# MarSaKi/VLN-BEVBert

Measured on AMD Instinct MI355X. Metric: pretrain_samples_per_sec, higher is better.
Workload: dtype bf16+fp32-residual

## Files before the change

include/bevbert_hip.h:

```cpp
#ifndef BEVBERT_HIP_H
#define BEVBERT_HIP_H

#include <stdint.h>

#ifdef __cplusplus
extern "C" {
#endif

typedef struct ihipStream_t* hipStream_t;

#define BEVBERT_F32 0
#define BEVBERT_BF16 1
#define BEVBERT_F16 2

const char* bevbert_last_error(void);
int bevbert_version(void);
int bevbert_hip_error_reset(void);
const char* bevbert_arch(void);
const char* bevbert_attn_last_path(int backward);
const char* bevbert_attn_plan(int B, int nh, int Lq, int Lk, int dtype, int impl, int has_key_mask, int has_bias,
                              float drop_p, int has_bits, int bits_ready, int want_dbias, int ncu, int backward);

int bevbert_bev_lift_bin(const float* depths, const float* T_c2w, const float* T_w2c, const float* S_w2c,
                         const float* pix_scale, int B, int V, int hw, float depth_scale, int dim, float res,
// ... 29 lines not shown
int bevbert_layernorm_bwd(const void* dy, const void* z, const float* mean, const float* rstd, const float* gamma,
                          void* dz, void* dx, float* dgamma, float* dbeta, float* dbias, float* workspace, int rows,
                          int H, int dtype, float drop_p, uint64_t seed, uint64_t offset, int accumulate,
                          hipStream_t stream);
int bevbert_layernorm_bwd_add(const void* dy, const void* z, const float* mean, const float* rstd, const float* gamma,
                              void* dz, void* dx, const void* dz_add, float* dgamma, float* dbeta, float* dbias,
                              float* workspace, int rows, int H, int dtype, float drop_p, uint64_t seed, uint64_t offset,
                              int accumulate, hipStream_t stream);
int bevbert_layernorm_res32_fwd(const void* x, const float* bias, const void* residual, int residual_dtype,
                                const float* gamma, const float* beta, void* y16, float* y32, float* z32, float* mean,
                                float* rstd, int rows, int H, float eps, float drop_p, uint64_t seed, uint64_t offset,
                                hipStream_t stream);
int bevbert_layernorm_res32_bwd(const void* dy16, const float* dy32, const float* z32, const float* mean,
                                const float* rstd, const float* gamma, void* dz, void* dx16, float* dgamma,
                                float* dbeta, float* dbias, float* workspace, int rows, int H, float drop_p, uint64_t seed,
                                uint64_t offset, int accumulate, int dz_dtype,
                                hipStream_t stream);
int64_t bevbert_colsum_workspace_floats(int total_cols);
int bevbert_colsum_partial_rows(int rows);
int bevbert_colsum_finalize(const float* partials, int nblocks, int nwhich, int C, float* out0, float* out1,
                            float* out2, int accumulate, hipStream_t stream);
int bevbert_colsum_partials(const void* dy, float* partials, int rows, int C, int dtype, hipStream_t stream);
int bevbert_multi_finalize(const void* tasks, int ntasks, hipStream_t stream);
int bevbert_multi_accum(const void* tasks, int ntasks, hipStream_t stream);

int bevbert_embed_sum_layernorm_fwd(const int64_t* ids, const void* word, const void* pos, const void* type_row,
                                    const float* gamma, const float* beta, void* y, void* z_out, float* mean,
                                    float* rstd, int rows, int L, int H, float eps, int dtype, float drop_p,
                                    uint64_t seed, uint64_t offset, hipStream_t stream);

int bevbert_embedding_grad(const int64_t* ids, const void* d, float* table_grad, int rows, int H, int padding_idx,
                           int dtype, hipStream_t stream);

int64_t bevbert_smallk_workspace_floats(int rows, int K, int H);
int bevbert_smallk_linear_layernorm_fwd(const float* feat, const float* weight, const float* bias, const float* gamma,
                                        const float* beta, const void* post1, const void* table, const int64_t* idx,
                                        void* y, float* mean, float* rstd, int rows, int K, int H, float eps, int dtype,
                                        hipStream_t stream);
int bevbert_smallk_linear_layernorm_bwd(const void* dy, const float* feat, const float* weight, const float* bias,
                                        const float* mean, const float* rstd, const float* gamma, float* dweight,
                                        float* dbias, float* dgamma, float* dbeta, float* workspace, int rows, int K,
                                        int H, int dtype, hipStream_t stream);

int bevbert_colsum_any(const void* dy, float* out, int rows, int C, int dtype, int accumulate, hipStream_t stream);

int bevbert_weighted_mean_fwd(const float* x, const float* w, const float* denom_dev, float denom, int n, float* out,
                              hipStream_t stream);
int bevbert_weighted_mean_bwd(const float* dout, const float* w, const float* denom_dev, float denom, int n, float* dx,
                              hipStream_t stream);

int bevbert_sem_select(const uint8_t* mask1, const uint8_t* mask2, int n, int cap, int classes, int64_t* idx, float* valid,
                       float* denom, hipStream_t stream);
int bevbert_bce_rows_fwd(const void* logits, const uint8_t* labels, const int64_t* idx, float* out, int rows, int C, int dtype,
                         hipStream_t stream);
int bevbert_bce_rows_bwd(const void* logits, const uint8_t* labels, const int64_t* idx, const float* g, void* dlogits, int rows,
                         int C, int dtype, hipStream_t stream);

int bevbert_graph_bias_fwd(const float* dists, const float* w, const float* b, float* out, int64_t n, hipStream_t stream);
int bevbert_graph_bias_bwd(const float* dbias, const float* dists, int layers, int B, int nh, int G, float* dw, float* db,
                           float* workspace , hipStream_t stream);

int bevbert_rows_gather(const void* src, const int64_t* ids, void* out, int rows, int H, int dtype, hipStream_t stream);
int bevbert_rows_scatter(const int64_t* ids, const void* d, void* out, int rows, int H, int dtype, int accumulate,
                         hipStream_t stream);

int bevbert_embedding_grad_sliced(const int64_t* ids, const void* d, float* partials, int rows, int H, int table_rows,
// ... 139 lines not shown
```

vln_bevbert_amd/csrc/rowops.hip:

```cpp
#include <math.h>
#include <type_traits>

#include "common.h"

template <typename T, int NV, bool GATHER>
__global__ __launch_bounds__(256) void ln_fwd_kernel(const T* __restrict__ x, const float* __restrict__ bias,
                                                     const T* __restrict__ residual, const float* __restrict__ gamma,
                                                     const float* __restrict__ beta, T* __restrict__ y,
                                                     T* __restrict__ z_out, float* __restrict__ mean_out,
                                                     float* __restrict__ rstd_out, int rows, float eps, float drop_p,
                                                     uint32_t drop_thr, uint32_t drop_key,
                                                     const int64_t* __restrict__ ids, const T* __restrict__ word,
                                                     const T* __restrict__ pos, const T* __restrict__ type_row, int L,
                                                     const uint32_t* __restrict__ salt) {
  constexpr int H = NV * 256;
  if (drop_p > 0.f) drop_key = bb_salted(drop_key, salt);
  const int lane = threadIdx.x & 63;
  const int row = blockIdx.x * 4 + (threadIdx.x >> 6);
  if (row >= rows) return;
  float4 v[NV];
  const float keep_scale = drop_p > 0.f ? 1.0f / (1.0f - drop_p) : 1.0f;
#pragma unroll
  for (int i = 0; i < NV; ++i) {
    const int col = (i * 64 + lane) * 4;
// ... 466 lines not shown
  const int r = blockIdx.x;
  const int e0 = rowptr[r], e1 = rowptr[r + 1];
  for (int c = threadIdx.x * 4; c < H; c += blockDim.x * 4) {
    float4 acc = make_float4(0.f, 0.f, 0.f, 0.f);
    for (int e = e0; e < e1; ++e) {
      const float ww = w[e];
      const float4 v = ld4<T>(src + (size_t)idx[e] * H + c);
      acc.x += ww * v.x; acc.y += ww * v.y; acc.z += ww * v.z; acc.w += ww * v.w;
    }
    st4<T>(out + (size_t)r * H + c, acc);
  }
}

template <typename T>
__global__ __launch_bounds__(256) void accum_partials_kernel(const T* __restrict__ partials, float* __restrict__ sink,
                                                             int S, size_t n4) {
  for (size_t i = (size_t)blockIdx.x * 256 + threadIdx.x; i < n4; i += (size_t)gridDim.x * 256) {
    float4 acc = *reinterpret_cast<const float4*>(sink + i * 4);
    for (int s = 0; s < S; ++s) {
      const float4 v = ld4<T>(partials + ((size_t)s * n4 + i) * 4);
      acc.x += v.x; acc.y += v.y; acc.z += v.z; acc.w += v.w;
    }
    *reinterpret_cast<float4*>(sink + i * 4) = acc;
  }
}

struct AccumTask {
  const void* partials;
  float* sink;
  unsigned long long n4_total;
  unsigned int off4, n4;
  int S, dtype;
};
template <typename T>
__device__ __forceinline__ void accum_task(const AccumTask& t) {
  const T* part = (const T*)t.partials;
  for (unsigned i = threadIdx.x; i < t.n4; i += 256) {
    float4 acc = *reinterpret_cast<const float4*>(t.sink + (size_t)i * 4);
    for (int s = 0; s < t.S; ++s) {
      const float4 v = ld4<T>(part + ((size_t)s * t.n4_total + t.off4 + i) * 4);
      acc.x += v.x; acc.y += v.y; acc.z += v.z; acc.w += v.w;
    }
    *reinterpret_cast<float4*>(t.sink + (size_t)i * 4) = acc;
  }
}
__global__ __launch_bounds__(256) void multi_accum_kernel(const AccumTask* __restrict__ tasks) {
  const AccumTask t = tasks[blockIdx.x];
  if (t.dtype == BB_BF16) accum_task<bf16_raw>(t);
  else accum_task<float>(t);
}

#define EG_MAXJ 4
template <typename T, typename TO = float, bool ACCUM = true>
__global__ __launch_bounds__(256) void embedding_grad_kernel(const int64_t* __restrict__ ids, const T* __restrict__ d,
                                                             TO* __restrict__ table_grad, int rows, int H,
                                                             int padding_idx) {
  __shared__ int s_flag;
  __shared__ float s_part[4][256 * EG_MAXJ];
  const int r = blockIdx.x, tid = threadIdx.x, lane = tid & 63, wave = tid >> 6;
  const int64_t id = ids[r];
  if (id == (int64_t)padding_idx) return;
  if (tid == 0) s_flag = 0;
  __syncthreads();
  int hit = 0;
  for (int i = tid; i < r; i += 256) hit |= (ids[i] == id);
  if (hit) s_flag = 1;
  __syncthreads();
  if (s_flag) return;
  float4 acc[EG_MAXJ];
#pragma unroll
  for (int j = 0; j < EG_MAXJ; ++j) acc[j] = make_float4(0.f, 0.f, 0.f, 0.f);
  const int span = rows - r, q = (span + 3) >> 2;
  const int lo = r + wave * q, hi = min(rows, lo + q);
  for (int base = lo; base < hi; base += 256) {
    unsigned long long bal[4];
#pragma unroll
    for (int u = 0; u < 4; ++u) {
      const int i = base + 64 * u + lane;
      bal[u] = __ballot(i < hi && ids[i] == id);
    }
#pragma unroll
    for (int u = 0; u < 4; ++u) {
      unsigned long long b = bal[u];
      while (b) {
        const int row = base + 64 * u + (__ffsll((long long)b) - 1);
        b &= b - 1;
#pragma unroll
        for (int j = 0; j < EG_MAXJ; ++j) {
          const int c = (lane + 64 * j) * 4;
          if (c < H) {
            const float4 v = ld4<T>(d + (size_t)row * H + c);
            acc[j].x += v.x; acc[j].y += v.y; acc[j].z += v.z; acc[j].w += v.w;
          }
        }
      }
    }
  }
#pragma unroll
  for (int j = 0; j < EG_MAXJ; ++j) *reinterpret_cast<float4*>(&s_part[wave][(lane + 64 * j) * 4]) = acc[j];
  __syncthreads();
  TO* dst = table_grad + (size_t)id * H;
  for (int c = tid * 4; c < H; c += 1024) {
    const float4 p0 = *reinterpret_cast<const float4*>(&s_part[0][c]), p1 = *reinterpret_cast<const float4*>(&s_part[1][c]);
    const float4 p2 = *reinterpret_cast<const float4*>(&s_part[2][c]), p3 = *reinterpret_cast<const float4*>(&s_part[3][c]);
    float4 t = make_float4(0.f, 0.f, 0.f, 0.f);
    if (ACCUM) t = ld4<TO>(dst + c);
    t.x += (p0.x + p1.x) + (p2.x + p3.x); t.y += (p0.y + p1.y) + (p2.y + p3.y);
    t.z += (p0.z + p1.z) + (p2.z + p3.z); t.w += (p0.w + p1.w) + (p2.w + p3.w);
    st4<TO>(dst + c, t);
  }
}

template <typename T>
__global__ __launch_bounds__(256) void rows_gather_kernel(const T* __restrict__ src, const int64_t* __restrict__ ids,
                                                          T* __restrict__ out, int H) {
  const int64_t id = ids[blockIdx.x];
  for (int c = threadIdx.x * 4; c < H; c += blockDim.x * 4)
    st4<T>(out + (size_t)blockIdx.x * H + c, ld4<T>(src + (size_t)id * H + c));
}

template <typename T>
__global__ __launch_bounds__(256) void embedding_grad_sliced_kernel(const int64_t* __restrict__ ids, const T* __restrict__ d,
                                                                    float* __restrict__ partials, int rows, int H,
                                                                    int rows_per_slice, int ntab) {
  const int t = blockIdx.x, s = blockIdx.y;
  const int r0 = s * rows_per_slice, r1 = min(rows, r0 + rows_per_slice);
  for (int c = threadIdx.x * 4; c < H; c += blockDim.x * 4) {
    float4 acc = make_float4(0.f, 0.f, 0.f, 0.f);
    for (int r = r0; r < r1; r += 4) {
      float4 v[4];
#pragma unroll
      for (int j = 0; j < 4; ++j) {
        v[j] = make_float4(0.f, 0.f, 0.f, 0.f);
        if (r + j < r1 && ids[r + j] == t) v[j] = ld4<T>(d + (size_t)(r + j) * H + c);
      }
#pragma unroll
      for (int j = 0; j < 4; ++j) { acc.x += v[j].x; acc.y += v[j].y; acc.z += v[j].z; acc.w += v[j].w; }
    }
    *reinterpret_cast<float4*>(partials + ((size_t)s * ntab + t) * H + c) = acc;
  }
}

__global__ __launch_bounds__(256) void sumsq_kernel(const float* __restrict__ g, size_t n4, float* __restrict__ partials) {
// ... 731 lines not shown
    hipLaunchKernelGGL((embedding_grad_kernel<float, float, true>), dim3(rows), dim3(256), 0, stream, ids, (const float*)d, (float*)out, rows, H, -1);
  else if (dtype == BB_F32)
    hipLaunchKernelGGL((embedding_grad_kernel<float, float, false>), dim3(rows), dim3(256), 0, stream, ids, (const float*)d, (float*)out, rows, H, -1);
  else if (dtype == BB_BF16 && accumulate)
    hipLaunchKernelGGL((embedding_grad_kernel<bf16_raw, bf16_raw, true>), dim3(rows), dim3(256), 0, stream, ids, (const bf16_raw*)d, (bf16_raw*)out, rows, H, -1);
  else if (dtype == BB_BF16)
    hipLaunchKernelGGL((embedding_grad_kernel<bf16_raw, bf16_raw, false>), dim3(rows), dim3(256), 0, stream, ids, (const bf16_raw*)d, (bf16_raw*)out, rows, H, -1);
  else {
    bb_set_error("rows_scatter: dtype %d unsupported", dtype);
    return BB_EUNSUPPORTED;
  }
  BB_CHECK_LAUNCH("rows_scatter");
  return BB_OK;
}

BEVBERT_API int bevbert_embedding_grad(const int64_t* ids, const void* d, float* table_grad, int rows, int H,
                                       int padding_idx, int dtype, hipStream_t stream) {
  BB_REQUIRE(H % 4 == 0 && H <= 256 * EG_MAXJ, "embedding_grad: H=%d must be a multiple of 4 and <= %d", H, 256 * EG_MAXJ);
  if (rows <= 0) return BB_OK;
  if (dtype == BB_F32)
    hipLaunchKernelGGL(embedding_grad_kernel<float>, dim3(rows), dim3(256), 0, stream, ids, (const float*)d, table_grad, rows, H,
                       padding_idx);
  else if (dtype == BB_BF16)
    hipLaunchKernelGGL(embedding_grad_kernel<bf16_raw>, dim3(rows), dim3(256), 0, stream, ids, (const bf16_raw*)d, table_grad,
                       rows, H, padding_idx);
  else {
    bb_set_error("embedding_grad: dtype %d unsupported", dtype);
    return BB_EUNSUPPORTED;
  }
  BB_CHECK_LAUNCH("embedding_grad");
  return BB_OK;
}

BEVBERT_API int bevbert_embedding_grad_sliced(const int64_t* ids, const void* d, float* partials, int rows, int H,
                                              int table_rows, int rows_per_slice, int dtype, hipStream_t stream) {
  BB_REQUIRE(H % 4 == 0, "embedding_grad_sliced: H=%d must be a multiple of 4", H);
  BB_REQUIRE(table_rows > 0 && rows_per_slice > 0 && rows > 0, "embedding_grad_sliced: empty problem (%d table rows, %d rows)",
             table_rows, rows);
  const int slices = (rows + rows_per_slice - 1) / rows_per_slice;
  BB_REQUIRE(slices <= 65535, "embedding_grad_sliced: %d slices exceed the grid limit", slices);
  const int nt = H / 4 < 256 ? ((H / 4 + 63) / 64) * 64 : 256;
  const dim3 grid(table_rows, slices);
  if (dtype == BB_F32)
    hipLaunchKernelGGL(embedding_grad_sliced_kernel<float>, grid, dim3(nt), 0, stream, ids, (const float*)d, partials, rows, H,
                       rows_per_slice, table_rows);
  else if (dtype == BB_BF16)
    hipLaunchKernelGGL(embedding_grad_sliced_kernel<bf16_raw>, grid, dim3(nt), 0, stream, ids, (const bf16_raw*)d, partials,
                       rows, H, rows_per_slice, table_rows);
  else {
    bb_set_error("embedding_grad_sliced: dtype %d unsupported", dtype);
    return BB_EUNSUPPORTED;
  }
  BB_CHECK_LAUNCH("embedding_grad_sliced");
  return BB_OK;
}

BEVBERT_API int bevbert_grad_norm_clip(const float* grads, int64_t n, float pre_scale, float max_norm,
                                       float* partials, float* scalars, hipStream_t stream) {
  BB_REQUIRE(n % 4 == 0, "grad_norm_clip: n must be a multiple of 4");
  hipLaunchKernelGGL(sumsq_kernel, dim3(1024), dim3(256), 0, stream, grads, (size_t)n / 4, partials);
  hipLaunchKernelGGL(clip_coef_kernel, dim3(1), dim3(256), 0, stream, partials, 1024, pre_scale, max_norm, scalars);
  BB_CHECK_LAUNCH("grad_norm_clip");
  return BB_OK;
}

BEVBERT_API int bevbert_adamw_step(float* params, const float* grads, float* exp_avg, float* exp_avg_sq,
// ... 56 lines not shown
```

vln_bevbert_amd/lib.py:

```python
import ctypes
import os
import re
import subprocess

import torch

_HERE = os.path.dirname(os.path.abspath(__file__))
LIB_PATH = os.path.join(_HERE, "libbevbert_hip.so")
CSRC = os.path.join(_HERE, "csrc")
EXTRA_FLAGS = {"attn_fwd4.hip": ["-fno-slp-vectorize"]}
SOURCES = ["splat.hip", "rowops.hip", "attn_simple.hip", "attn_f32.hip", "attn_mfma.hip", "attn_bwd1.hip", "attn_fwd2.hip", "attn_fwd4.hip", "attn_bwd2.hip", "attn_bwd3.hip", "attn_small.hip", "attn_short.hip", "smallk.hip", "sap_loss.hip", "graph_nav.hip", "nav_expert.hip", "waypoint.hip", "gemm.hip", "capi.hip"]
HEADER = os.path.join(os.path.dirname(_HERE), "include", "bevbert_hip.h")

F32, BF16, F16 = 0, 1, 2
_DT = {torch.float32: F32, torch.bfloat16: BF16, torch.float16: F16}


class BevBertHipError(RuntimeError):
    pass


def dtype_code(t):
    try:
        return _DT[t.dtype if torch.is_tensor(t) else t]
# ... 30 lines not shown


def header_symbols():
    with open(HEADER) as f:
        return sorted(set(re.findall(r"\b(bevbert_\w+)\s*\(", f.read())))


_lib = None
_P, _I, _I64, _U64, _F = ctypes.c_void_p, ctypes.c_int, ctypes.c_int64, ctypes.c_uint64, ctypes.c_float

_PROTOS = {
    "bevbert_bev_lift_bin": [_P, _P, _P, _P, _P, _I, _I, _I, _F, _I, _F, _F, _P, _P, _P, _P],
    "bevbert_bev_bin_points": [_P, _P, _I, _I, _I, _F, _F, _P, _P, _P, _P],
    "bevbert_bev_splat_mean": [_P, _I, _P, _P, _P, _I, _I, _I, _I, _I, _P, _P, _I, _P, _P, _P, _I, _P],
    "bevbert_attn_fwd": [_P, _P, _P, _P, _P, _P, _P, _P, _I, _I, _I, _I, _I, _F, _I, _I, _F, _U64, _U64, _P, _I, _P],
    "bevbert_attn_drop_bits": [_P, _I, _I, _I, _I, _F, _U64, _U64, _P],
    "bevbert_attn_bwd": [_P, _P, _P, _P, _P, _P, _P, _P, _P, _P, _P, _P, _P, _P, _I, _I, _I, _I, _I, _F, _I, _I, _F,
                         _U64, _U64, _P, _P],
    "bevbert_bias_dropout_residual_layernorm_fwd": [_P, _P, _P, _P, _P, _P, _P, _P, _P, _I, _I, _F, _I, _F, _U64,
                                                    _U64, _P],
    "bevbert_layernorm_post_fwd": [_P, _P, _P, _P, _P, _P, _P, _P, _P, _P, _I, _I, _F, _I, _P],
    "bevbert_layernorm_bwd": [_P, _P, _P, _P, _P, _P, _P, _P, _P, _P, _P, _I, _I, _I, _F, _U64, _U64, _I, _P],
    "bevbert_layernorm_res32_fwd": [_P, _P, _P, _I, _P, _P, _P, _P, _P, _P, _P, _I, _I, _F, _F, _U64, _U64, _P],
    "bevbert_layernorm_res32_bwd": [_P, _P, _P, _P, _P, _P, _P, _P, _P, _P, _P, _P, _I, _I, _F, _U64, _U64, _I, _I, _P],
    "bevbert_colsum_any": [_P, _P, _I, _I, _I, _I, _P],
    "bevbert_sem_select": [_P, _P, _I, _I, _I, _P, _P, _P, _P],
    "bevbert_bce_rows_fwd": [_P, _P, _P, _P, _I, _I, _I, _P],
    "bevbert_bce_rows_bwd": [_P, _P, _P, _P, _P, _I, _I, _I, _P],
    "bevbert_weighted_mean_fwd": [_P, _P, _P, _F, _I, _P, _P],
    "bevbert_weighted_mean_bwd": [_P, _P, _P, _F, _I, _P, _P],
    "bevbert_layernorm_bwd_add": [_P, _P, _P, _P, _P, _P, _P, _P, _P, _P, _P, _P, _I, _I, _I, _F, _U64, _U64, _I, _P],
    "bevbert_embed_sum_layernorm_fwd": [_P, _P, _P, _P, _P, _P, _P, _P, _P, _P, _I, _I, _I, _F, _I, _F, _U64, _U64, _P],
    "bevbert_embedding_grad": [_P, _P, _P, _I, _I, _I, _I, _P],
    "bevbert_rows_gather": [_P, _P, _P, _I, _I, _I, _P],
    "bevbert_graph_bias_fwd": [_P, _P, _P, _P, _I64, _P],
    "bevbert_graph_bias_bwd": [_P, _P, _I, _I, _I, _I, _P, _P, _P, _P],
    "bevbert_smallk_linear_layernorm_fwd": [_P] * 11 + [_I, _I, _I, _F, _I, _P],
    "bevbert_smallk_linear_layernorm_bwd": [_P] * 12 + [_I, _I, _I, _I, _P],
    "bevbert_rows_scatter": [_P, _P, _P, _I, _I, _I, _I, _P],
    "bevbert_embedding_grad_sliced": [_P, _P, _P, _I, _I, _I, _I, _I, _P],
    "bevbert_bias_gelu_fwd": [_P, _P, _P, _I, _I, _I, _P],
    "bevbert_bias_gelu_bwd": [_P, _P, _P, _P, _P, _P, _I, _I, _I, _I, _P],
    "bevbert_bias_relu_fwd": [_P, _P, _P, _I, _I, _I, _P],
    "bevbert_bias_relu_bwd": [_P, _P, _P, _P, _P, _P, _I, _I, _I, _I, _P],
    "bevbert_colsum": [_P, _P, _P, _I, _I, _I, _I, _P],
    "bevbert_segment_wsum": [_P, _P, _P, _P, _P, _I, _I, _I, _P],
    "bevbert_grad_norm_clip": [_P, _I64, _F, _F, _P, _P, _P],
    "bevbert_adamw_step": [_P, _P, _P, _P, _P, _P, _P, _I64, _P, _P, _F, _F, _F, _F, _F, _P],
    "bevbert_set_step_salt": [_P],
    "bevbert_colsum_partials": [_P, _P, _I, _I, _I, _P],
    "bevbert_multi_finalize": [_P, _I, _P],
    "bevbert_multi_accum": [_P, _I, _P],
    "bevbert_cast_f32": [_P, _P, _I64, _I, _P],
    "bevbert_zero": [_P, _I64, _P],
    "bevbert_accum_partials": [_P, _P, _I, _I64, _I, _P],
    "bevbert_dropout_keep_mask": [_P, _I64, _F, _U64, _U64, _P],
    "bevbert_gemm": [_P, _P, _P, _P, _I, _I, _I, _I, _I, _I64, _I64, _I64, _I, _I64, _I64, _I64, _I, _I, _I, _F, _P,
                     _I64, _I, _P],
    "bevbert_colsum_finalize": [_P, _I, _I, _I, _P, _P, _P, _I, _P],
    "bevbert_dropout_add": [_P, _P, _P, _I64, _I, _I, _F, _U64, _U64, _P],
    "bevbert_gm_update": [_P] * 10 + [_I, _I, _P, _P, _P],
    "bevbert_gm_nav_vars": [_P] * 7 + [_I, _I, _I] + [_P] * 7,
    "bevbert_gm_bev_select": [_P, _P, _I, _I, _P, _P, _P, _P, _P],
    "bevbert_gm_gather_views": [_P, _P, _P, _P, _I, _I64, _P],
    "bevbert_gm_embed_update": [_P] * 9 + [_I, _I, _I, _I, _P],
    "bevbert_gm_node_embeds": [_P, _P, _P, _P, _P, _I, _I, _I, _P, _P],
# ... 102 lines not shown
```

vln_bevbert_amd/ops_rowops.py:

```python
import math

import torch

from . import lib
from .lib import dtype_code, ptr, stream
from .ops_core import RT, _compute, _f32, _mark_touched, _sink, call
from .ops_reduce import ReduceQueue, WgradStream, _on_launch_stream, _partial_rows


def embedding_grad_small(ids, d, sink, table_rows):
    rows, H = d.shape
    per = 64
    while (rows + per - 1) // per * table_rows > 4096:
        per *= 2
    slices = (rows + per - 1) // per
    part = RT.scratch.alloc(slices * table_rows * H * 4, d.device)
    call("bevbert_embedding_grad_sliced", ptr(ids), ptr(d), part, rows, H, table_rows, per, dtype_code(d), stream())
    ReduceQueue.add(part, slices, 1, table_rows * H, (sink.data_ptr(), None, None))


def _ln_param_dests(gamma, beta, bias, H, dev):
    outs = []
    for p in (gamma, beta, bias):
        if p is None:
            outs.append((None, None, 0))
        elif p is bias and not getattr(p, "requires_grad", True):
            outs.append((None, None, None))
        elif _sink(p) is not None:
            outs.append((_sink(p), None, 1))
            _mark_touched(p)
        else:
            t = torch.empty(H, dtype=torch.float32, device=dev)
            outs.append((t, t, 0))
    (dg, rg, ag), (db, rb, ab), (dbi, rbi, abi) = outs
    assert ag == ab and (bias is None or abi is None or abi == ag), "mixed arena / plain parameters in one LayerNorm"
    return (dg, db, dbi), (rg, rb, rbi), ag


def _ln_bwd_call(entry, head, mid, tail, dests, accumulate, rows, H, dev, ws=None):
    if accumulate == 1 and WgradStream.DEFER_FINALIZE and dev.type == "cuda":
        nb = _partial_rows(rows)
        part = RT.scratch.alloc(nb * 3 * H * 4, dev)
        call(entry, *head, None, None, None, part, *mid, 1, *tail, stream())
        ReduceQueue.add(part, nb, 3, H, tuple(ptr(d) for d in dests))
    else:
        if ws is None:
            ws = RT.workspace(dev, lib.load().bevbert_colsum_workspace_floats(3 * H))
        call(entry, *head, *(ptr(d) for d in dests), ptr(ws), *mid, accumulate, *tail, stream())


class _BiasDropResLN(torch.autograd.Function):
# ... 393 lines not shown
    @staticmethod
    def backward(ctx, g):
        logits, labels, idx = ctx.saved_tensors
        rows, C = logits.shape
        dx = torch.empty_like(logits)
        call("bevbert_bce_rows_bwd", ptr(logits), ptr(labels), ptr(idx), ptr(g.contiguous().float()), ptr(dx), rows, C,
             dtype_code(logits), stream())
        return dx, None, None


def bce_rows(logits, labels, idx=None):
    return _BceRows.apply(logits, labels, idx)


@torch.no_grad()
def sem_select(mask1, mask2, cap, classes):
    m1 = mask1.reshape(-1).contiguous()
    m2 = None if mask2 is None else mask2.reshape(-1).contiguous()
    assert m1.dtype in (torch.bool, torch.uint8) and (m2 is None or (m2.dtype in (torch.bool, torch.uint8) and m2.numel() == m1.numel()))
    dev = m1.device
    idx = torch.empty(cap, dtype=torch.int64, device=dev)
    valid = torch.empty(cap, dtype=torch.float32, device=dev)
    denom = torch.empty((), dtype=torch.float32, device=dev)
    call("bevbert_sem_select", ptr(m1), ptr(m2), m1.numel(), cap, classes, ptr(idx), ptr(valid), ptr(denom), stream())
    return idx, valid, denom


class _TakeRows(torch.autograd.Function):

    @staticmethod
    def forward(ctx, x, idx, idx2=None):
        assert x.is_contiguous() and idx.dtype == torch.int64 and idx.is_contiguous()
        H = x.shape[-1]
        outs = []
        for ix in (idx, idx2):
            if ix is None:
                continue
            o = torch.empty((ix.numel(), H), dtype=x.dtype, device=x.device)
            call("bevbert_rows_gather", ptr(x), ptr(ix), ptr(o), ix.numel(), H, dtype_code(x), stream())
            outs.append(o)
        ctx.save_for_backward(idx, idx2)
        ctx.shape = x.shape
        ctx.set_materialize_grads(False)
        return tuple(outs) if idx2 is not None else outs[0]

    @staticmethod
    def backward(ctx, *grads):
        idx, idx2 = ctx.saved_tensors
        some = next((g for g in grads if g is not None), None)
        if some is None:
            return None, None, None
        H = ctx.shape[-1]
        dx = torch.empty(ctx.shape, dtype=some.dtype, device=some.device)
        call("bevbert_zero", ptr(dx), dx.numel() * dx.element_size(), stream())
        first = True
        for ix, g in zip((idx, idx2), grads):
            if ix is None or g is None:
                continue
            g = g.contiguous()
            call("bevbert_rows_scatter", ptr(ix), ptr(g), ptr(dx), ix.numel(), H, dtype_code(g), 0 if first else 1, stream())
            first = False
        return dx, None, None


def take_rows(x, idx, idx2=None):
    return _TakeRows.apply(x.contiguous(), idx, idx2)


def bias_gelu(x, bias):
    return _BiasGelu.apply(x, bias)


def bias_relu(x, bias):
    return _BiasGelu.apply(x, bias, "relu")


class _EmbedLN(torch.autograd.Function):
    @staticmethod
    def forward(ctx, ids, word, pos, typ, gamma, beta, eps, type_index, word_c, pos_c, typ_c, pad_idx=-1):
        B, L = ids.shape
        H = word_c.shape[1]
        rows = B * L
        y = torch.empty(B, L, H, dtype=word_c.dtype, device=ids.device)
        need_grad = any(ctx.needs_input_grad)
        z = torch.empty_like(y) if need_grad else None
        mean = torch.empty(rows, dtype=torch.float32, device=ids.device) if need_grad else None
        rstd = torch.empty(rows, dtype=torch.float32, device=ids.device) if need_grad else None
        ids = ids.contiguous()
        call("bevbert_embed_sum_layernorm_fwd", ptr(ids), ptr(word_c), ptr(pos_c), ptr(typ_c[type_index]),
             ptr(_f32(gamma)), ptr(_f32(beta)), ptr(y), ptr(z), ptr(mean), ptr(rstd), rows, L, H, float(eps),
             dtype_code(y), 0.0, 0, 0, stream())
        ctx.save_for_backward(ids, z, mean, rstd)
        ctx.params = (word, pos, typ, gamma, beta, type_index, int(pad_idx))
        return y

    @staticmethod
    def backward(ctx, dy):
        ids, z, mean, rstd = ctx.saved_tensors
        word, pos, typ, gamma, beta, type_index, pad_idx = ctx.params
        B, L = ids.shape
        H = z.shape[-1]
        rows = B * L
        dy = dy.contiguous()
        dz = torch.empty_like(dy)
        ws = RT.workspace(dy.device, lib.load().bevbert_colsum_workspace_floats(3 * H))
        sg, sb = _sink(gamma), _sink(beta)
        assert (sg is None) == (sb is None)
        styp = _sink(typ)[type_index] if (sg is not None and typ.requires_grad and _sink(typ) is not None) else None
        if sg is not None:
            _mark_touched(gamma); _mark_touched(beta)
            if styp is not None:
                _mark_touched(typ)
            rg = rb = None
        else:
            rg = torch.empty(H, dtype=torch.float32, device=dy.device)
            rb = torch.empty(H, dtype=torch.float32, device=dy.device)
        _ln_bwd_call("bevbert_layernorm_bwd", (ptr(dy), ptr(z), ptr(mean), ptr(rstd), ptr(_f32(gamma)), ptr(dz), None),
                     (rows, H, dtype_code(dy), 0.0, 0, 0), (), (sg, sb, styp) if sg is not None else (rg, rb, None),
                     1 if sg is not None else 0, rows, H, dy.device, ws)
        dz2 = dz.reshape(rows, H)
        dzf = dz2

        def word_grad(t):
            call("bevbert_embedding_grad", ptr(ids), ptr(dz2), ptr(t), rows, H, pad_idx, dtype_code(dz2), stream())

        def pos_grad(t):
            call("bevbert_colsum_any", ptr(dz2), ptr(t), B, L * H, dtype_code(dz2), 1, stream())

        def typ_grad(t):
            call("bevbert_colsum_any", ptr(dz2), ptr(t[type_index]), rows, H, dtype_code(dz2), 1, stream())

        makers = ((word, word_grad), (pos, pos_grad), (typ, typ_grad))
        outs, deferred = [], []
        for p, make in makers:
            if not p.requires_grad:
                outs.append(None)
            elif p is typ and styp is not None:
                outs.append(None)
            elif _sink(p) is not None:
                _mark_touched(p)
                deferred.append((make, _sink(p)))
                outs.append(None)
            else:
                t = torch.zeros(p.shape, dtype=torch.float32, device=dy.device)
                make(t)
                outs.append(t.to(p.dtype))
        if deferred:
            WgradStream.submit(dy.device, lambda: [m(t) for m, t in deferred], dz2, dzf, ids, dy)
        return (None, outs[0], outs[1], outs[2], rg, rb, None, None, None, None, None, None)


def embed_sum_layernorm(ids, word, pos, typ, gamma, beta, eps, type_index=0, padding_idx=None):
    return _EmbedLN.apply(ids, word, pos, typ, gamma, beta, eps, type_index, _compute(word), _compute(pos),
                          _compute(typ), -1 if padding_idx is None else int(padding_idx))


class SegmentCSR:

    def __init__(self, rowptr, idx, w, n_src, device, capacity=None):
        self.n_out, self.n_src = len(rowptr) - 1, int(n_src)
        self.capacity = int(capacity) if capacity is not None else len(idx)
        pack, packw = self._pack(rowptr, idx, w)
        di = torch.from_numpy(pack).to(device, non_blocking=True)
        dw = torch.from_numpy(packw).to(device, non_blocking=True)
        self._di, self._dw = di, dw
        n0, n1, n2 = self.n_out + 1, self.capacity, self.n_src + 1
        self.rowptr, self.idx = di[:n0], di[n0:n0 + n1]
        self.t_rowptr, self.t_idx = di[n0 + n1:n0 + n1 + n2], di[n0 + n1 + n2:]
        self.w, self.t_w = dw[:n1], dw[n1:]

    def _pack(self, rowptr, idx, w):
        import numpy as np
        rowptr = np.asarray(rowptr, dtype=np.int32)
        idx = np.asarray(idx, dtype=np.int32)
        w = np.asarray(w, dtype=np.float32)
        assert len(rowptr) == self.n_out + 1 and len(idx) <= self.capacity, "segment CSR does not fit its buffers"
        out_of_e = np.repeat(np.arange(self.n_out, dtype=np.int32), np.diff(rowptr))
        order = np.argsort(idx, kind="stable")
        t_rowptr = np.zeros(self.n_src + 1, dtype=np.int32)
        np.add.at(t_rowptr, idx + 1, 1)
        t_rowptr = np.cumsum(t_rowptr).astype(np.int32)
# ... 105 lines not shown
```

Before: 3697.

## Add sorted-index embedding grad path and unroll multi-accum partial reduction

Adds an index-building kernel that computes, per row of ids, first-occurrence flags, sorted offsets, counts and a permutation list. New indexed embedding-grad and row-scatter kernels use that index to sum only the duplicate rows, replacing the quadratic scan over earlier rows. The indexed path is behind an environment flag that is off by default. Separately, the multi-task accumulation kernel now processes two float4 groups and four slices per iteration to increase memory-level parallelism, at the cost of more registers.

```diff
diff --git a/include/bevbert_hip.h b/include/bevbert_hip.h
--- a/include/bevbert_hip.h
+++ b/include/bevbert_hip.h
@@ -85,6 +85,12 @@
 int bevbert_embedding_grad(const int64_t* ids, const void* d, float* table_grad, int rows, int H, int padding_idx,
                            int dtype, hipStream_t stream);
 
+int bevbert_embedding_index(const int64_t* ids, int rows, int padding_idx, int* index, hipStream_t stream);
+int bevbert_embedding_grad_indexed(const int64_t* ids, const int* index, const void* d, float* table_grad, int rows, int H,
+                                   int dtype, hipStream_t stream);
+int bevbert_rows_scatter_indexed(const int64_t* ids, const int* index, const void* d, void* out, int rows, int H, int dtype,
+                                 int accumulate, hipStream_t stream);
+
 int64_t bevbert_smallk_workspace_floats(int rows, int K, int H);
 int bevbert_smallk_linear_layernorm_fwd(const float* feat, const float* weight, const float* bias, const float* gamma,
                                         const float* beta, const void* post1, const void* table, const int64_t* idx,
diff --git a/vln_bevbert_amd/csrc/rowops.hip b/vln_bevbert_amd/csrc/rowops.hip
--- a/vln_bevbert_amd/csrc/rowops.hip
+++ b/vln_bevbert_amd/csrc/rowops.hip
@@ -522,17 +522,40 @@
   unsigned int off4, n4;
   int S, dtype;
 };
+template <typename T, int NI>
+__device__ __forceinline__ void accum_groups(const T* __restrict__ part, size_t stride, float* __restrict__ sink, int S) {
+  float4 acc[NI];
+#pragma unroll
+  for (int k = 0; k < NI; ++k) acc[k] = *reinterpret_cast<const float4*>(sink + (size_t)k * 1024);
+  int s = 0;
+  for (; s + 4 <= S; s += 4) {
+    float4 v[4][NI];
+#pragma unroll
+    for (int u = 0; u < 4; ++u)
+#pragma unroll
+      for (int k = 0; k < NI; ++k) v[u][k] = ld4<T>(part + (size_t)(s + u) * stride + (size_t)k * 1024);
+#pragma unroll
+    for (int u = 0; u < 4; ++u)
+#pragma unroll
+      for (int k = 0; k < NI; ++k) { acc[k].x += v[u][k].x; acc[k].y += v[u][k].y; acc[k].z += v[u][k].z; acc[k].w += v[u][k].w; }
+  }
+  for (; s < S; ++s) {
+    float4 v[NI];
+#pragma unroll
+    for (int k = 0; k < NI; ++k) v[k] = ld4<T>(part + (size_t)s * stride + (size_t)k * 1024);
+#pragma unroll
+    for (int k = 0; k < NI; ++k) { acc[k].x += v[k].x; acc[k].y += v[k].y; acc[k].z += v[k].z; acc[k].w += v[k].w; }
+  }
+#pragma unroll
+  for (int k = 0; k < NI; ++k) *reinterpret_cast<float4*>(sink + (size_t)k * 1024) = acc[k];
+}
 template <typename T>
 __device__ __forceinline__ void accum_task(const AccumTask& t) {
-  const T* part = (const T*)t.partials;
-  for (unsigned i = threadIdx.x; i < t.n4; i += 256) {
-    float4 acc = *reinterpret_cast<const float4*>(t.sink + (size_t)i * 4);
-    for (int s = 0; s < t.S; ++s) {
-      const float4 v = ld4<T>(part + ((size_t)s * t.n4_total + t.off4 + i) * 4);
-      acc.x += v.x; acc.y += v.y; acc.z += v.z; acc.w += v.w;
-    }
-    *reinterpret_cast<float4*>(t.sink + (size_t)i * 4) = acc;
-  }
+  const T* part = (const T*)t.partials + (size_t)t.off4 * 4;
+  const size_t stride = (size_t)t.n4_total * 4;
+  unsigned i = threadIdx.x;
+  for (; i + 256 < t.n4; i += 512) accum_groups<T, 2>(part + (size_t)i * 4, stride, t.sink + (size_t)i * 4, t.S);
+  if (i < t.n4) accum_groups<T, 1>(part + (size_t)i * 4, stride, t.sink + (size_t)i * 4, t.S);
 }
 __global__ __launch_bounds__(256) void multi_accum_kernel(const AccumTask* __restrict__ tasks) {
   const AccumTask t = tasks[blockIdx.x];
@@ -541,6 +564,22 @@
 }
 
 #define EG_MAXJ 4
+template <typename TO, bool ACCUM>
+__device__ __forceinline__ void eg_fold(float (*s_part)[256 * EG_MAXJ], const float4 (&acc)[EG_MAXJ], TO* __restrict__ dst,
+                                        int H, int tid, int lane, int wave) {
+#pragma unroll
+  for (int j = 0; j < EG_MAXJ; ++j) *reinterpret_cast<float4*>(&s_part[wave][(lane + 64 * j) * 4]) = acc[j];
+  __syncthreads();
+  for (int c = tid * 4; c < H; c += 1024) {
+    const float4 p0 = *reinterpret_cast<const float4*>(&s_part[0][c]), p1 = *reinterpret_cast<const float4*>(&s_part[1][c]);
+    const float4 p2 = *reinterpret_cast<const float4*>(&s_part[2][c]), p3 = *reinterpret_cast<const float4*>(&s_part[3][c]);
+    float4 t = make_float4(0.f, 0.f, 0.f, 0.f);
+    if (ACCUM) t = ld4<TO>(dst + c);
+    t.x += (p0.x + p1.x) + (p2.x + p3.x); t.y += (p0.y + p1.y) + (p2.y + p3.y);
+    t.z += (p0.z + p1.z) + (p2.z + p3.z); t.w += (p0.w + p1.w) + (p2.w + p3.w);
+    st4<TO>(dst + c, t);
+  }
+}
 template <typename T, typename TO = float, bool ACCUM = true>
 __global__ __launch_bounds__(256) void embedding_grad_kernel(const int64_t* __restrict__ ids, const T* __restrict__ d,
                                                              TO* __restrict__ table_grad, int rows, int H,
@@ -586,19 +625,90 @@
       }
     }
   }
-#pragma unroll
-  for (int j = 0; j < EG_MAXJ; ++j) *reinterpret_cast<float4*>(&s_part[wave][(lane + 64 * j) * 4]) = acc[j];
+  eg_fold<TO, ACCUM>(s_part, acc, table_grad + (size_t)id * H, H, tid, lane, wave);
+}
+
+#define EG_INDEX_MAX_ROWS 8192
+__global__ __launch_bounds__(256) void embedding_index_kernel(const int64_t* __restrict__ ids, int rows, int padding_idx,
+                                                              int* __restrict__ index) {
+  __shared__ int s_cnt[3][4][64];
+  const int lane = threadIdx.x & 63, wave = __builtin_amdgcn_readfirstlane(threadIdx.x >> 6);
+  const int r = blockIdx.x * 64 + lane;
+  const int64_t id = ids[r < rows ? r : rows - 1];
+  const int q = (rows + 3) >> 2, j0 = wave * q, j1 = min(rows, j0 + q);
+  int less = 0, before = 0, same = 0;
+#pragma unroll 8
+  for (int j = j0; j < j1; ++j) {
+    const int64_t v = ids[j];
+    const int e = v == id;
+    less += v < id;
+    same += e;
+    before += e & (j < r);
+  }
+  s_cnt[0][wave][lane] = less; s_cnt[1][wave][lane] = before; s_cnt[2][wave][lane] = same;
   __syncthreads();
-  TO* dst = table_grad + (size_t)id * H;
-  for (int c = tid * 4; c < H; c += 1024) {
-    const float4 p0 = *reinterpret_cast<const float4*>(&s_part[0][c]), p1 = *reinterpret_cast<const float4*>(&s_part[1][c]);
-    const float4 p2 = *reinterpret_cast<const float4*>(&s_part[2][c]), p3 = *reinterpret_cast<const float4*>(&s_part[3][c]);
-    float4 t = make_float4(0.f, 0.f, 0.f, 0.f);
-    if (ACCUM) t = ld4<TO>(dst + c);
-    t.x += (p0.x + p1.x) + (p2.x + p3.x); t.y += (p0.y + p1.y) + (p2.y + p3.y);
-    t.z += (p0.z + p1.z) + (p2.z + p3.z); t.w += (p0.w + p1.w) + (p2.w + p3.w);
-    st4<TO>(dst + c, t);
-  }
+  if (wave != 0 || r >= rows) return;
+  less = (s_cnt[0][0][lane] + s_cnt[0][1][lane]) + (s_cnt[0][2][lane] + s_cnt[0][3][lane]);
+  before = (s_cnt[1][0][lane] + s_cnt[1][1][lane]) + (s_cnt[1][2][lane] + s_cnt[1][3][lane]);
+  same = (s_cnt[2][0][lane] + s_cnt[2][1][lane]) + (s_cnt[2][2][lane] + s_cnt[2][3][lane]);
+  index[r] = before == 0 && id != (int64_t)padding_idx;
+  index[rows + r] = less + before;
+  index[2 * rows + r] = same;
+  index[3 * rows + less + before] = r;
+}
+
+template <typename T, typename TO, bool ACCUM>
+__global__ __launch_bounds__(256) void embedding_grad_indexed_kernel(const int64_t* __restrict__ ids, const int* __restrict__ index,
+                                                                     const T* __restrict__ d, TO* __restrict__ table_grad,
+                                                                     int rows, int H) {
+  __shared__ float s_part[4][256 * EG_MAXJ];
+  const int r = blockIdx.x;
+  if (!index[r]) return;
+  const int tid = threadIdx.x, lane = tid & 63, wave = __builtin_amdgcn_readfirstlane(tid >> 6);
+  const int* __restrict__ list = index + 3 * (size_t)rows + index[rows + r];
+  const int n = index[2 * rows + r];
+  const int span = rows - r, q = (span + 3) >> 2;
+  const int lo = r + wave * q, hi = min(rows, lo + q);
+  int a = 0, b = 0;
+  for (int k = 0; k < n; k += 64) {
+    const bool in = k + lane < n;
+    const int row = in ? list[k + lane] : 0;
+    a += __popcll(__ballot(in && row < lo));
+    b += __popcll(__ballot(in && row < hi));
+  }
+  float4 acc[EG_MAXJ];
+#pragma unroll
+  for (int j = 0; j < EG_MAXJ; ++j) acc[j] = make_float4(0.f, 0.f, 0.f, 0.f);
+  int e = a;
+  for (; e + 4 <= b; e += 4) {
+    float4 v[4][EG_MAXJ];
+#pragma unroll
+    for (int u = 0; u < 4; ++u) {
+      const int row = list[e + u];
+#pragma unroll
+      for (int j = 0; j < EG_MAXJ; ++j) {
+        const int c = (lane + 64 * j) * 4;
+        v[u][j] = make_float4(0.f, 0.f, 0.f, 0.f);
+        if (c < H) v[u][j] = ld4<T>(d + (size_t)row * H + c);
+      }
+    }
+#pragma unroll
+    for (int u = 0; u < 4; ++u)
+#pragma unroll
+      for (int j = 0; j < EG_MAXJ; ++j) { acc[j].x += v[u][j].x; acc[j].y += v[u][j].y; acc[j].z += v[u][j].z; acc[j].w += v[u][j].w; }
+  }
+  for (; e < b; ++e) {
+    const int row = list[e];
+#pragma unroll
+    for (int j = 0; j < EG_MAXJ; ++j) {
+      const int c = (lane + 64 * j) * 4;
+      if (c < H) {
+        const float4 v = ld4<T>(d + (size_t)row * H + c);
+        acc[j].x += v.x; acc[j].y += v.y; acc[j].z += v.z; acc[j].w += v.w;
+      }
+    }
+  }
+  eg_fold<TO, ACCUM>(s_part, acc, table_grad + (size_t)ids[r] * H, H, tid, lane, wave);
 }
 
 template <typename T>
@@ -1396,6 +1506,55 @@
   return BB_OK;
 }
 
+BEVBERT_API int bevbert_embedding_index(const int64_t* ids, int rows, int padding_idx, int* index, hipStream_t stream) {
+  BB_REQUIRE(rows <= EG_INDEX_MAX_ROWS, "embedding_index: %d rows exceed %d (use the scanning kernels)", rows, EG_INDEX_MAX_ROWS);
+  if (rows <= 0) return BB_OK;
+  BB_REQUIRE(ids != nullptr && index != nullptr, "embedding_index: null ids or index");
+  hipLaunchKernelGGL(embedding_index_kernel, dim3((rows + 63) / 64), dim3(256), 0, stream, ids, rows, padding_idx, index);
+  BB_CHECK_LAUNCH("embedding_index");
+  return BB_OK;
+}
+
+BEVBERT_API int bevbert_embedding_grad_indexed(const int64_t* ids, const int* index, const void* d, float* table_grad, int rows,
+                                               int H, int dtype, hipStream_t stream) {
+  BB_REQUIRE(H % 4 == 0 && H <= 256 * EG_MAXJ, "embedding_grad_indexed: H=%d must be a multiple of 4 and <= %d", H, 256 * EG_MAXJ);
+  BB_REQUIRE(rows <= EG_INDEX_MAX_ROWS, "embedding_grad_indexed: %d rows exceed %d", rows, EG_INDEX_MAX_ROWS);
+  if (rows <= 0) return BB_OK;
+  BB_REQUIRE(index != nullptr, "embedding_grad_indexed: null index");
+  if (dtype == BB_F32)
+    hipLaunchKernelGGL((embedding_grad_indexed_kernel<float, float, true>), dim3(rows), dim3(256), 0, stream, ids, index, (const float*)d, table_grad, rows, H);
+  else if (dtype == BB_BF16)
+    hipLaunchKernelGGL((embedding_grad_indexed_kernel<bf16_raw, float, true>), dim3(rows), dim3(256), 0, stream, ids, index, (const bf16_raw*)d, table_grad, rows, H);
+  else {
+    bb_set_error("embedding_grad_indexed: dtype %d unsupported", dtype);
+    return BB_EUNSUPPORTED;
+  }
+  BB_CHECK_LAUNCH("embedding_grad_indexed");
+  return BB_OK;
+}
+
+BEVBERT_API int bevbert_rows_scatter_indexed(const int64_t* ids, const int* index, const void* d, void* out, int rows, int H,
+                                             int dtype, int accumulate, hipStream_t stream) {
+  BB_REQUIRE(H % 4 == 0 && H <= 256 * EG_MAXJ, "rows_scatter_indexed: H=%d must be a multiple of 4 and <= %d", H, 256 * EG_MAXJ);
+  BB_REQUIRE(rows <= EG_INDEX_MAX_ROWS, "rows_scatter_indexed: %d rows exceed %d", rows, EG_INDEX_MAX_ROWS);
+  if (rows <= 0) return BB_OK;
+  BB_REQUIRE(index != nullptr, "rows_scatter_indexed: null index");
+  if (dtype == BB_F32 && accumulate)
+    hipLaunchKernelGGL((embedding_grad_indexed_kernel<float, float, true>), dim3(rows), dim3(256), 0, stream, ids, index, (const float*)d, (float*)out, rows, H);
+  else if (dtype == BB_F32)
+    hipLaunchKernelGGL((embedding_grad_indexed_kernel<float, float, false>), dim3(rows), dim3(256), 0, stream, ids, index, (const float*)d, (float*)out, rows, H);
+  else if (dtype == BB_BF16 && accumulate)
+    hipLaunchKernelGGL((embedding_grad_indexed_kernel<bf16_raw, bf16_raw, true>), dim3(rows), dim3(256), 0, stream, ids, index, (const bf16_raw*)d, (bf16_raw*)out, rows, H);
+  else if (dtype == BB_BF16)
+    hipLaunchKernelGGL((embedding_grad_indexed_kernel<bf16_raw, bf16_raw, false>), dim3(rows), dim3(256), 0, stream, ids, index, (const bf16_raw*)d, (bf16_raw*)out, rows, H);
+  else {
+    bb_set_error("rows_scatter_indexed: dtype %d unsupported", dtype);
+    return BB_EUNSUPPORTED;
+  }
+  BB_CHECK_LAUNCH("rows_scatter_indexed");
+  return BB_OK;
+}
+
 BEVBERT_API int bevbert_embedding_grad_sliced(const int64_t* ids, const void* d, float* partials, int rows, int H,
                                               int table_rows, int rows_per_slice, int dtype, hipStream_t stream) {
   BB_REQUIRE(H % 4 == 0, "embedding_grad_sliced: H=%d must be a multiple of 4", H);
diff --git a/vln_bevbert_amd/lib.py b/vln_bevbert_amd/lib.py
--- a/vln_bevbert_amd/lib.py
+++ b/vln_bevbert_amd/lib.py
@@ -86,6 +86,9 @@
     "bevbert_layernorm_bwd_add": [_P, _P, _P, _P, _P, _P, _P, _P, _P, _P, _P, _P, _I, _I, _I, _F, _U64, _U64, _I, _P],
     "bevbert_embed_sum_layernorm_fwd": [_P, _P, _P, _P, _P, _P, _P, _P, _P, _P, _I, _I, _I, _F, _I, _F, _U64, _U64, _P],
     "bevbert_embedding_grad": [_P, _P, _P, _I, _I, _I, _I, _P],
+    "bevbert_embedding_index": [_P, _I, _I, _P, _P],
+    "bevbert_embedding_grad_indexed": [_P, _P, _P, _P, _I, _I, _I, _P],
+    "bevbert_rows_scatter_indexed": [_P, _P, _P, _P, _I, _I, _I, _I, _P],
     "bevbert_rows_gather": [_P, _P, _P, _I, _I, _I, _P],
     "bevbert_graph_bias_fwd": [_P, _P, _P, _P, _I64, _P],
     "bevbert_graph_bias_bwd": [_P, _P, _I, _I, _I, _I, _P, _P, _P, _P],
diff --git a/vln_bevbert_amd/ops_rowops.py b/vln_bevbert_amd/ops_rowops.py
--- a/vln_bevbert_amd/ops_rowops.py
+++ b/vln_bevbert_amd/ops_rowops.py
@@ -1,4 +1,5 @@
 import math
+import os as _os
 
 import torch
 
@@ -17,6 +18,19 @@
     part = RT.scratch.alloc(slices * table_rows * H * 4, d.device)
     call("bevbert_embedding_grad_sliced", ptr(ids), ptr(d), part, rows, H, table_rows, per, dtype_code(d), stream())
     ReduceQueue.add(part, slices, 1, table_rows * H, (sink.data_ptr(), None, None))
+
+
+EMBGRAD_INDEX = _os.environ.get("BEVBERT_EMBGRAD_INDEX", "0") == "1"
+EMBGRAD_INDEX_MAX_ROWS = 8192
+
+
+def match_index(ids, padding_idx=-1):
+    rows = ids.numel()
+    if not EMBGRAD_INDEX or not 0 < rows <= EMBGRAD_INDEX_MAX_ROWS:
+        return None
+    index = torch.empty(4 * rows, dtype=torch.int32, device=ids.device)
+    call("bevbert_embedding_index", ptr(ids), rows, int(padding_idx), ptr(index), stream())
+    return index
 
 
 def _ln_param_dests(gamma, beta, bias, H, dev):
@@ -476,21 +490,23 @@
     def forward(ctx, x, idx, idx2=None):
         assert x.is_contiguous() and idx.dtype == torch.int64 and idx.is_contiguous()
         H = x.shape[-1]
-        outs = []
+        outs, index = [], []
         for ix in (idx, idx2):
             if ix is None:
+                index.append(None)
                 continue
             o = torch.empty((ix.numel(), H), dtype=x.dtype, device=x.device)
             call("bevbert_rows_gather", ptr(x), ptr(ix), ptr(o), ix.numel(), H, dtype_code(x), stream())
             outs.append(o)
-        ctx.save_for_backward(idx, idx2)
+            index.append(match_index(ix) if ctx.needs_input_grad[0] and H <= 1024 else None)
+        ctx.save_for_backward(idx, idx2, *index)
         ctx.shape = x.shape
         ctx.set_materialize_grads(False)
         return tuple(outs) if idx2 is not None else outs[0]
 
     @staticmethod
     def backward(ctx, *grads):
-        idx, idx2 = ctx.saved_tensors
+        idx, idx2, *index = ctx.saved_tensors
         some = next((g for g in grads if g is not None), None)
         if some is None:
             return None, None, None
@@ -498,11 +514,17 @@
         dx = torch.empty(ctx.shape, dtype=some.dtype, device=some.device)
         call("bevbert_zero", ptr(dx), dx.numel() * dx.element_size(), stream())
         first = True
-        for ix, g in zip((idx, idx2), grads):
-            if ix is None or g is None:
+        grads = iter(grads)
+        for ix, mi in zip((idx, idx2), index):
+            g = None if ix is None else next(grads)
+            if g is None:
                 continue
             g = g.contiguous()
-            call("bevbert_rows_scatter", ptr(ix), ptr(g), ptr(dx), ix.numel(), H, dtype_code(g), 0 if first else 1, stream())
+            if mi is not None:
+                call("bevbert_rows_scatter_indexed", ptr(ix), ptr(mi), ptr(g), ptr(dx), ix.numel(), H, dtype_code(g),
+                     0 if first else 1, stream())
+            else:
+                call("bevbert_rows_scatter", ptr(ix), ptr(g), ptr(dx), ix.numel(), H, dtype_code(g), 0 if first else 1, stream())
             first = False
         return dx, None, None
 
@@ -534,13 +556,14 @@
         call("bevbert_embed_sum_layernorm_fwd", ptr(ids), ptr(word_c), ptr(pos_c), ptr(typ_c[type_index]),
              ptr(_f32(gamma)), ptr(_f32(beta)), ptr(y), ptr(z), ptr(mean), ptr(rstd), rows, L, H, float(eps),
              dtype_code(y), 0.0, 0, 0, stream())
-        ctx.save_for_backward(ids, z, mean, rstd)
+        index = match_index(ids, pad_idx) if ctx.needs_input_grad[1] and H <= 1024 else None
+        ctx.save_for_backward(ids, z, mean, rstd, index)
         ctx.params = (word, pos, typ, gamma, beta, type_index, int(pad_idx))
         return y
 
     @staticmethod
     def backward(ctx, dy):
-        ids, z, mean, rstd = ctx.saved_tensors
+        ids, z, mean, rstd, index = ctx.saved_tensors
         word, pos, typ, gamma, beta, type_index, pad_idx = ctx.params
         B, L = ids.shape
         H = z.shape[-1]
@@ -566,7 +589,10 @@
         dzf = dz2
 
         def word_grad(t):
-            call("bevbert_embedding_grad", ptr(ids), ptr(dz2), ptr(t), rows, H, pad_idx, dtype_code(dz2), stream())
+            if index is not None:
+                call("bevbert_embedding_grad_indexed", ptr(ids), ptr(index), ptr(dz2), ptr(t), rows, H, dtype_code(dz2), stream())
+            else:
+                call("bevbert_embedding_grad", ptr(ids), ptr(dz2), ptr(t), rows, H, pad_idx, dtype_code(dz2), stream())
 
         def pos_grad(t):
             call("bevbert_colsum_any", ptr(dz2), ptr(t), B, L * H, dtype_code(dz2), 1, stream())
@@ -590,7 +616,7 @@
                 make(t)
                 outs.append(t.to(p.dtype))
         if deferred:
-            WgradStream.submit(dy.device, lambda: [m(t) for m, t in deferred], dz2, dzf, ids, dy)
+            WgradStream.submit(dy.device, lambda: [m(t) for m, t in deferred], dz2, dzf, ids, index, dy)
         return (None, outs[0], outs[1], outs[2], rg, rb, None, None, None, None, None, None)
 
 
```

Result: no change. 3668 (-0.8%).
